# lizuoyue/torch-ngp

Measured on AMD Instinct MI355X. Metric: train-step rays/sec (fwd+bwd) on 800×800 Lego; 1/2/4/8 MI355X, higher is better.
Workload: dtype fp16

## Files before the change

torch-ngp_amd/csrc/ngp_head.h:

```cpp
#pragma once
#include "ngp_common.h"
#include "ngp_step.h"

#include <cfloat>


namespace ngp_head {

using ngp_step::StepState;

constexpr int kMaxBoxes = 8;
constexpr int kMaxTensors = 8;
constexpr uint32_t kMaxMapRes = 128;

NGP_DEV uint32_t mix32(uint32_t x) {
    x ^= x >> 16; x *= 0x7feb352du;
    x ^= x >> 15; x *= 0x846ca68bu;
    x ^= x >> 16;
    return x;
}
NGP_DEV uint32_t rng_u32(uint32_t seed, uint32_t a, uint32_t b, uint32_t c) {
    return mix32(seed ^ mix32(a + 0x9e3779b9u * mix32(b ^ mix32(c + 0x85ebca6bu))));
}
NGP_DEV float rng_unit(uint32_t seed, uint32_t a, uint32_t b, uint32_t c) {
// ... 311 lines not shown
#else
    const uint2 w = __builtin_bit_cast(uint2, g);
    return ((w.x | w.y) & 0x7fff7fffu) == 0u && m.x == 0.0f && m.y == 0.0f && m.z == 0.0f && m.w == 0.0f &&
           v.x == 0.0f && v.y == 0.0f && v.z == 0.0f && v.w == 0.0f;
#endif
}
constexpr uint32_t kAdamThreads = 256, kAdamChunk = kAdamThreads * 8;
template <int U = 2>
NGP_DEV void adam_sweep(const TensorList& tl, StepState* __restrict__ st, const AdamArgs& aa, uint32_t blk,
                        uint32_t nblk, uint32_t tid) {
    constexpr uint32_t kChunk = kAdamThreads * 4 * U;
    const ngp_step::AdamConsts ac = ngp_step::adam_consts(st, aa.base_lr, aa.beta1, aa.beta2, aa.iters,
                                                          aa.grad_mult);
    const bool skip = st->found_inf != 0 || ac.inv_bad;
    if (blk == 0 && tid == 0) {
        if (ac.inv_bad) st->found_inf = 1;
        if (aa.defer_end) st->end_pending = 1;
    }
    typedef _Float16 half4 __attribute__((ext_vector_type(4)));
    const bool shadow_all = (aa.zero_grads & 2) != 0;
    auto adam1 = [&](float& p, float& m, float& v, float gh) {
        ngp_step::adam_update(p, m, v, gh, ac, aa.beta1, aa.beta2, aa.eps);
    };
    const uint64_t total = tl.start[tl.n];
    const uint64_t nchunks = (total + kChunk - 1) / kChunk;
    for (uint64_t c = blk; c < nchunks; c += nblk) {
        const uint64_t c0 = c * kChunk, c1 = min(c0 + kChunk, total);
        const int k = find_tensor(tl, c0);
        if (find_tensor(tl, c1 - 1) == k && c1 - tl.start[k] <= tl.size[k]) {
            const uint64_t base = c0 - tl.start[k] + tid * 4;
            float4 pv[U], mv[U], vv[U];
            half4 gh[U];
            bool in[U];
#pragma unroll
            for (int u = 0; u < U; ++u) {
                const uint64_t off = base + u * (kChunk / U);
                in[u] = c0 + (off - (c0 - tl.start[k])) < c1;
                const uint64_t lo = in[u] ? off : c0 - tl.start[k];
                pv[u] = *reinterpret_cast<const float4*>(tl.p[k] + lo);
                mv[u] = *reinterpret_cast<const float4*>(tl.m[k] + lo);
                vv[u] = *reinterpret_cast<const float4*>(tl.v[k] + lo);
                gh[u] = *reinterpret_cast<const half4*>(tl.g[k] + lo);
            }
#pragma unroll
            for (int u = 0; u < U; ++u) {
                if (!in[u]) continue;
                const uint64_t off = base + u * (kChunk / U);
                const bool upd = !skip && !adam_idle(mv[u], vv[u], gh[u]);
                if (upd) {
                    adam1(pv[u].x, mv[u].x, vv[u].x, (float)gh[u][0]);
                    adam1(pv[u].y, mv[u].y, vv[u].y, (float)gh[u][1]);
                    adam1(pv[u].z, mv[u].z, vv[u].z, (float)gh[u][2]);
                    adam1(pv[u].w, mv[u].w, vv[u].w, (float)gh[u][3]);
                    *reinterpret_cast<float4*>(tl.p[k] + off) = pv[u];
                    *reinterpret_cast<float4*>(tl.m[k] + off) = mv[u];
                    *reinterpret_cast<float4*>(tl.v[k] + off) = vv[u];
                }
                if (tl.ph[k] && (upd || shadow_all))
                    *reinterpret_cast<half4*>(tl.ph[k] + off) =
                        half4{(ngp_half)pv[u].x, (ngp_half)pv[u].y, (ngp_half)pv[u].z, (ngp_half)pv[u].w};
                if (aa.zero_grads && grad_set(gh[u])) *reinterpret_cast<half4*>(tl.g[k] + off) = half4{0, 0, 0, 0};
            }
            continue;
        }
        for (uint64_t i = c0 + tid; i < c1; i += kAdamThreads) {
            const int kk = find_tensor(tl, i);
            const uint64_t off = i - tl.start[kk];
            if (off >= tl.size[kk]) continue;
            float p = tl.p[kk][off];
            if (!skip) {
                float m = tl.m[kk][off], v = tl.v[kk][off];
                adam1(p, m, v, (float)tl.g[kk][off]);
                tl.p[kk][off] = p;
                tl.m[kk][off] = m;
                tl.v[kk][off] = v;
            }
            if (tl.ph[kk] && (!skip || shadow_all)) tl.ph[kk][off] = (ngp_half)p;
            if (aa.zero_grads) tl.g[kk][off] = (ngp_half)0.0f;
        }
    }
}

template <int U>
NGP_DEV void adam_sweep_pipe(const TensorList& tl, StepState* __restrict__ st, const AdamArgs& aa, uint32_t blk,
                             uint32_t nblk, uint32_t tid) {
    constexpr uint32_t kChunk = kAdamThreads * 4 * U;
    typedef _Float16 half4 __attribute__((ext_vector_type(4)));
    const ngp_step::AdamConsts ac = ngp_step::adam_consts(st, aa.base_lr, aa.beta1, aa.beta2, aa.iters,
                                                          aa.grad_mult);
    const bool skip = st->found_inf != 0 || ac.inv_bad;
    if (blk == 0 && tid == 0) {
        if (ac.inv_bad) st->found_inf = 1;
        if (aa.defer_end) st->end_pending = 1;
    }
    const bool shadow_all = (aa.zero_grads & 2) != 0;
    const uint64_t total = tl.start[tl.n];
    const uint64_t nchunks = (total + kChunk - 1) / kChunk;
    struct Buf {
        float4 p[U], m[U], v[U];
        half4 g[U];
    };
    auto whole = [&](uint64_t c) {
        const uint64_t c0 = c * kChunk, c1 = min(c0 + kChunk, total);
        const int k = find_tensor(tl, c0);
        return find_tensor(tl, c1 - 1) == k && c1 - tl.start[k] <= tl.size[k] ? k : -1;
    };
    auto ld_f4 = [](const float* q) { return *reinterpret_cast<const float4*>(q); };
    auto st_f4 = [](float* q, float4 x) { *reinterpret_cast<float4*>(q) = x; };
    auto load = [&](uint64_t c, int k, Buf& b) {
        const uint64_t c0 = c * kChunk, c1 = min(c0 + kChunk, total), first = c0 - tl.start[k];
#pragma unroll
        for (int u = 0; u < U; ++u) {
            const uint64_t off = first + tid * 4 + u * (kChunk / U);
            const uint64_t lo = off + tl.start[k] < c1 ? off : first;
            b.p[u] = ld_f4(tl.p[k] + lo);
            b.m[u] = ld_f4(tl.m[k] + lo);
            b.v[u] = ld_f4(tl.v[k] + lo);
            b.g[u] = *reinterpret_cast<const half4*>(tl.g[k] + lo);
        }
    };
    auto apply = [&](uint64_t c, int k, Buf& b) {
        const uint64_t c0 = c * kChunk, c1 = min(c0 + kChunk, total), first = c0 - tl.start[k];
#pragma unroll
        for (int u = 0; u < U; ++u) {
            const uint64_t off = first + tid * 4 + u * (kChunk / U);
            if (off + tl.start[k] >= c1) continue;
            const bool upd = !skip && !adam_idle(b.m[u], b.v[u], b.g[u]);
            if (upd) {
                ngp_step::adam_update(b.p[u].x, b.m[u].x, b.v[u].x, (float)b.g[u][0], ac, aa.beta1, aa.beta2, aa.eps);
                ngp_step::adam_update(b.p[u].y, b.m[u].y, b.v[u].y, (float)b.g[u][1], ac, aa.beta1, aa.beta2, aa.eps);
                ngp_step::adam_update(b.p[u].z, b.m[u].z, b.v[u].z, (float)b.g[u][2], ac, aa.beta1, aa.beta2, aa.eps);
                ngp_step::adam_update(b.p[u].w, b.m[u].w, b.v[u].w, (float)b.g[u][3], ac, aa.beta1, aa.beta2, aa.eps);
                st_f4(tl.p[k] + off, b.p[u]);
                st_f4(tl.m[k] + off, b.m[u]);
                st_f4(tl.v[k] + off, b.v[u]);
            }
            if (tl.ph[k] && (upd || shadow_all))
                *reinterpret_cast<half4*>(tl.ph[k] + off) =
                    half4{(ngp_half)b.p[u].x, (ngp_half)b.p[u].y, (ngp_half)b.p[u].z, (ngp_half)b.p[u].w};
            if (aa.zero_grads && grad_set(b.g[u])) *reinterpret_cast<half4*>(tl.g[k] + off) = half4{0, 0, 0, 0};
        }
    };
    auto seam = [&](uint64_t c) {
        const uint64_t c0 = c * kChunk, c1 = min(c0 + kChunk, total);
        for (uint64_t i = c0 + tid; i < c1; i += kAdamThreads) {
            const int kk = find_tensor(tl, i);
            const uint64_t off = i - tl.start[kk];
            if (off >= tl.size[kk]) continue;
            float p = tl.p[kk][off];
            if (!skip) {
                float m = tl.m[kk][off], v = tl.v[kk][off];
                ngp_step::adam_update(p, m, v, (float)tl.g[kk][off], ac, aa.beta1, aa.beta2, aa.eps);
                tl.p[kk][off] = p;
                tl.m[kk][off] = m;
                tl.v[kk][off] = v;
            }
            if (tl.ph[kk] && (!skip || shadow_all)) tl.ph[kk][off] = (ngp_half)p;
            if (aa.zero_grads) tl.g[kk][off] = (ngp_half)0.0f;
        }
    };
    auto at = [](uint64_t i) { return i; };
    Buf a{}, b{};
    uint64_t c = blk;
    int ka = c < nchunks ? whole(at(c)) : -1;
    if (ka >= 0) load(at(c), ka, a);
    while (c < nchunks) {
        const uint64_t cn = c + nblk;
        const int kb = cn < nchunks ? whole(at(cn)) : -1;
        if (kb >= 0) load(at(cn), kb, b);
        if (ka >= 0) apply(at(c), ka, a);
        else seam(at(c));
        a = b;
        ka = kb;
        c = cn;
    }
}

}
```

torch-ngp_amd/csrc/raymarching.hip:

```cpp
#include "ffmlp_pack.h"
#include "ngp_common.h"
#include "ngp_dpp.h"
#include "ngp_head.h"
#include "ngp_render.h"
#include "ngp_step.h"

#include <algorithm>
#include <cfloat>

namespace {

constexpr float kSQRT3 = 1.7320508075688772f;
constexpr float kRPI = 0.3183098861837907f;

NGP_DEV float clampf(float x, float lo, float hi) { return fminf(hi, fmaxf(lo, x)); }
NGP_DEV float signf(float x) { return copysignf(1.0f, x); }

NGP_DEV int frexp_level(float mx, int max_level) {
    int e = 0;
    if (mx != 0.0f) e = (int)((__float_as_uint(mx) >> 23) & 0xffu) - 126;
    return min(max_level, max(0, e));
}

NGP_DEV uint32_t expand_bits(uint32_t v) {
// ... 504 lines not shown
    if (mine && off < k.max_steps) {
        float tj = ta;
        uint64_t m = mine;
        for (uint32_t j = 0; m && off < k.max_steps; ++j, tj = ch.step(tj)) {
            if ((m >> j) & 1ull) {
                ts[off++] = tj;
                m &= m - 1;
            }
        }
    }
    return total < k.max_steps ? total : k.max_steps;
}

template <bool ONE_LEVEL, typename OCC>
NGP_DEV uint32_t march_ray_wave(const Ray& r, const MarchConst& k, const OCC& occ, float t0, float far,
                                float* __restrict__ ts) {
    if (!(t0 < far)) return 0;
    if (k.dt_gamma == 0.0f) {
        const float delta = clampf(0.0f, k.dt_min, k.dt_max);
        const float ulp_far = __uint_as_float(((__float_as_uint(far) >> 23) & 0xffu) << 23) * 1.1920929e-7f;
        const double smin = (double)delta - (double)ulp_far;
        if (smin > 0.0) {
            const double kest = ceil(((double)far - (double)t0) / smin) + 2.0;
            const uint32_t L = (uint32_t)ceil(kest / 64.0);
            if (L <= 64) return march_ray_segmented<ONE_LEVEL>(r, k, occ, ChainConst{t0, delta}, far, L, ts);
        }
    } else if (k.dt_gamma > 0.0f) {
        ChainGamma ch;
        ch.k = k;
        const uint32_t K = chain_records(t0, far, k, ch.rec);
        if (K != kInf) {
            ch.nrec = ngp_div_up(K, kRecStride);
            const uint32_t L = kRecStride * ngp_div_up(ngp_div_up(K, 64u), kRecStride);
            return march_ray_segmented<ONE_LEVEL>(r, k, occ, ch, far, L > 0 ? L : kRecStride, ts);
        }
    }
    uint32_t n = 0;
    if ((threadIdx.x & 63) == 0) n = march_ray_train<ONE_LEVEL>(r, k, occ, t0, far, ts);
    return (uint32_t)__builtin_amdgcn_readlane((int)n, 0);
}

NGP_DEV void emit_sample(const float* __restrict__ rays_o, const float* __restrict__ rays_d, const MarchConst& k,
                         const float* __restrict__ nears, const float* __restrict__ noises,
                         const float* __restrict__ ts, uint32_t rn, uint32_t kk, size_t p, float* __restrict__ xyzs,
                         float* __restrict__ dirs, float* __restrict__ deltas) {
    const float* row = ts + (size_t)rn * k.max_steps;
    const float t = row[kk];
    const float tp = row[kk ? kk - 1 : 0u];
    const float nr = nears[rn], nz = noises[rn];
    const float prev = kk == 0 ? ray_t0(nr, nz, k) : tp + clampf(tp * k.dt_gamma, k.dt_min, k.dt_max);
    const float ox = rays_o[rn * 3], oy = rays_o[rn * 3 + 1], oz = rays_o[rn * 3 + 2];
    const float dx = rays_d[rn * 3], dy = rays_d[rn * 3 + 1], dz = rays_d[rn * 3 + 2];
    const float dt = clampf(t * k.dt_gamma, k.dt_min, k.dt_max);
    xyzs[p * 3 + 0] = clampf(fmaf(t, dx, ox), -k.bound, k.bound);
    xyzs[p * 3 + 1] = clampf(fmaf(t, dy, oy), -k.bound, k.bound);
    xyzs[p * 3 + 2] = clampf(fmaf(t, dz, oz), -k.bound, k.bound);
    dirs[p * 3 + 0] = dx;
    dirs[p * 3 + 1] = dy;
    dirs[p * 3 + 2] = dz;
    deltas[p * 2 + 0] = dt;
    deltas[p * 2 + 1] = (t + dt) - prev;
}

struct MarchAdam {
    ngp_head::TensorList tl;
    ngp_head::AdamArgs aa;
    ngp_step::StepState* st;
    uint4* clear;
    uint32_t clear16;
    bool emit_launch;
};
constexpr uint32_t kMarchAdamWaves = 4;

constexpr uint32_t kEmitMaxBlockRays = 64;
struct MarchEmit {
    uint32_t* ticket;
    uint32_t* error;
    unsigned long long* words;
    int32_t* counter;
    float *xyzs, *dirs, *deltas;
    uint32_t M, rb;
};

NGP_DEV unsigned long long agent_load_u64(const unsigned long long* p) {
    return __hip_atomic_load(p, __ATOMIC_RELAXED, __HIP_MEMORY_SCOPE_AGENT);
}

template <uint32_t MW>
__global__ void __launch_bounds__(kSegThreads)
k_march_train(const float* __restrict__ rays_o, const float* __restrict__ rays_d,
              const uint8_t* __restrict__ grid, const uint8_t* __restrict__ img, OccLayout L,
              MarchConst k, uint32_t N, const float* __restrict__ nears, const float* __restrict__ fars,
              const float* __restrict__ noises, int32_t* __restrict__ rays, float* __restrict__ ts,
              const int32_t* __restrict__ counter, uint32_t* __restrict__ scan, MarchAdam ma, MarchEmit me) {
    extern __shared__ uint4 dyn[];
    __shared__ uint32_t s_ticket, s_base0, s_arrive, s_ready, s_first;
    __shared__ uint32_t s_off[kEmitMaxBlockRays + 1];
    const bool emit = me.ticket != nullptr;
    if (blockIdx.x == 0 && threadIdx.x == 0) scan[0] = (uint32_t)counter[0];
    if (emit && threadIdx.x == 0) {
        s_ticket = atomicAdd(me.ticket, 1u);
        s_base0 = (uint32_t)counter[0];
        s_arrive = 0;
        s_ready = 0;
    }
    uint32_t* sum = reinterpret_cast<uint32_t*>(dyn);
    uint32_t* pre = sum + 4 * L.ngroups;
    const bool lds = L.ngroups > 0 && load_occ_index(img, L, dyn);
    if (emit) __syncthreads();
    const uint32_t wave = threadIdx.x >> 6;
    if (MW < kSegWaves && wave >= MW) {
        constexpr uint32_t kVirt = (kSegWaves - MW) / 4;
        if (blockIdx.x == 0 && wave == MW)
            for (uint32_t i = threadIdx.x & 63u; i < ma.clear16; i += 64) ma.clear[i] = uint4{0u, 0u, 0u, 0u};
        ngp_head::adam_sweep_pipe<2>(ma.tl, ma.st, ma.aa, blockIdx.x * kVirt + (wave - MW) / 4,
                                                    gridDim.x * kVirt, threadIdx.x & 255u);
        return;
    }
    const OccLds occ_lds{sum, pre, reinterpret_cast<const uint8_t*>(pre + L.ngroups)};
    const OccGlobal occ_glb{grid};
    const uint32_t G = gridDim.x;
    const uint32_t rank = emit ? s_ticket % G : blockIdx.x, epoch1 = emit ? s_ticket / G + 1u : 0u;
    const uint32_t n0 = emit ? rank * me.rb : 0u, n1 = emit ? min(N, n0 + me.rb) : N;
    const uint32_t lane = threadIdx.x & 63;
    for (uint32_t n = emit ? n0 + wave : blockIdx.x * MW + wave; n < n1; n += emit ? MW : G * MW) {
        const Ray r = load_ray(rays_o, rays_d, n);
        const float t0 = ray_t0(nears[n], noises[n], k);
        const float far = fars[n];
        float* row = ts + (size_t)n * k.max_steps;
        uint32_t cnt;
        if (lds) {
            cnt = k.C == 1 ? march_ray_wave<true>(r, k, occ_lds, t0, far, row)
                           : march_ray_wave<false>(r, k, occ_lds, t0, far, row);
        } else {
            cnt = k.C == 1 ? march_ray_wave<true>(r, k, occ_glb, t0, far, row)
                           : march_ray_wave<false>(r, k, occ_glb, t0, far, row);
        }
        if (lane == 0) {
            rays[n * 3 + 0] = (int32_t)n;
            rays[n * 3 + 2] = (int32_t)cnt;
            scan[4 + n] = cnt;
            if (emit) s_off[n - n0] = cnt;
        }
    }
    if (!emit) return;
    asm volatile("s_waitcnt vmcnt(0) lgkmcnt(0)" ::: "memory");
    __builtin_amdgcn_fence(__ATOMIC_RELEASE, "workgroup");
    uint32_t last = 0;
    if (lane == 0) last = atomicAdd(&s_arrive, 1u) == MW - 1 ? 1u : 0u;
    last = (uint32_t)__builtin_amdgcn_readfirstlane((int)last);
    const uint32_t nb = n1 > n0 ? n1 - n0 : 0u;
    if (last) {
        __builtin_amdgcn_fence(__ATOMIC_ACQUIRE, "workgroup");
        const uint32_t c = lane < nb ? s_off[lane] : 0u;
        uint32_t incl = c;
#pragma unroll
        for (uint32_t o = 1; o < 64; o <<= 1) {
            const uint32_t u = __shfl_up(incl, o, 64);
            if (lane >= o) incl += u;
        }
        const uint32_t total = (uint32_t)__builtin_amdgcn_readlane((int)incl, 63);
        if (lane == 0)
            __hip_atomic_store(me.words + rank, ((unsigned long long)epoch1 << 32) | total, __ATOMIC_RELAXED,
                               __HIP_MEMORY_SCOPE_AGENT);
        uint32_t part = 0;
        bool lost = false;
        for (uint32_t p = lane; p < rank; p += 64) {
            unsigned long long v = agent_load_u64(me.words + p);
            for (uint32_t spin = 0; (uint32_t)(v >> 32) != epoch1 && spin < (1u << 20); ++spin) {
                __builtin_amdgcn_s_sleep(2);
                v = agent_load_u64(me.words + p);
            }
            lost |= (uint32_t)(v >> 32) != epoch1;
            part += (uint32_t)v;
        }
        if (__ballot(lost) && lane == 0) atomicOr(me.error, 1u);
#pragma unroll
        for (uint32_t o = 32; o > 0; o >>= 1) part += __shfl_xor(part, o, 64);
        if (lane < nb) s_off[lane] = incl - c;
        if (lane == 0) {
            s_off[nb] = total;
            s_first = s_base0 + part;
            if (rank == G - 1) {
                me.counter[0] = (int32_t)(s_base0 + part + total);
                me.counter[1] += (int32_t)N;
            }
        }
        __builtin_amdgcn_fence(__ATOMIC_RELEASE, "workgroup");
        if (lane == 0) __hip_atomic_store(&s_ready, 1u, __ATOMIC_RELAXED, __HIP_MEMORY_SCOPE_WORKGROUP);
    } else {
        for (uint32_t spin = 0; __hip_atomic_load(&s_ready, __ATOMIC_RELAXED, __HIP_MEMORY_SCOPE_WORKGROUP) == 0u &&
                                spin < (1u << 22); ++spin)
            __builtin_amdgcn_s_sleep(1);
        if (__hip_atomic_load(&s_ready, __ATOMIC_RELAXED, __HIP_MEMORY_SCOPE_WORKGROUP) == 0u && lane == 0)
            atomicOr(me.error, 2u);
        __builtin_amdgcn_fence(__ATOMIC_ACQUIRE, "workgroup");
    }
    const uint32_t base = s_first, btotal = s_off[nb];
    const uint32_t t = threadIdx.x;
    for (uint32_t i = t; i < nb; i += 64 * MW) rays[(size_t)(n0 + i) * 3 + 1] = (int32_t)(base + s_off[i]);
    for (uint32_t j = t; j < btotal; j += 64 * MW) {
        uint32_t lo = 0, hi = nb;
        while (hi - lo > 1) {
            const uint32_t mid = (lo + hi) >> 1;
            if (s_off[mid] <= j) lo = mid; else hi = mid;
        }
        if (base + s_off[lo + 1] > me.M) continue;
        emit_sample(rays_o, rays_d, k, nears, noises, ts, n0 + lo, j - s_off[lo], (size_t)base + j, me.xyzs,
                    me.dirs, me.deltas);
    }
}
static_assert((kSegWaves - kMarchAdamWaves) % 4 == 0, "Adam waves form 256-thread virtual blocks");

struct EmitTail {
    ngp_step::StepState* st;
    bool end;
    ngp_step::ScalerArgs sa;
    const float* loss_ray;
    uint32_t n_rays, groups;
    ngp_pack::PackJobs jobs;
};

__global__ void __launch_bounds__(kMarchThreads)
k_march_emit(const float* __restrict__ rays_o, const float* __restrict__ rays_d, MarchConst k,
             uint32_t N, uint32_t M, const float* __restrict__ nears, const float* __restrict__ noises,
             const float* __restrict__ ts, float* __restrict__ xyzs, float* __restrict__ dirs,
             float* __restrict__ deltas, int32_t* __restrict__ rays, const uint32_t* __restrict__ scan,
             int32_t* __restrict__ counter, EmitTail tail) {
    const bool has_tail = tail.st != nullptr;
    if (has_tail && blockIdx.y == 0) {
        if (blockIdx.x == 0) {
            if (tail.end && tail.st->end_pending)
                ngp_step::step_end_block(tail.st, tail.sa, nullptr, nullptr, tail.loss_ray, tail.n_rays);
        } else if (blockIdx.x - 1 < (uint32_t)tail.jobs.n) {
            const ngp_pack::PackJob& j = tail.jobs.job[blockIdx.x - 1];
            ngp_pack::build_frags(j.image, j.w, j.m, j.transposed != 0);
        }
        return;
    }
    if (blockIdx.x >= tail.groups) return;
    __shared__ uint32_t off[kMarchThreads + 1];
    __shared__ uint32_t lds_waves[kMarchThreads / 64];
    const uint32_t* __restrict__ counts = scan + 4;
    const uint32_t n0 = blockIdx.x * kMarchThreads;
    uint32_t part = 0;
    for (uint32_t i0 = threadIdx.x; i0 < n0; i0 += 8 * kMarchThreads) {
        uint32_t v[8];
#pragma unroll
        for (int u = 0; u < 8; ++u) {
            const uint32_t i = i0 + u * kMarchThreads;
            v[u] = counts[i < n0 ? i : 0u];
        }
#pragma unroll
        for (int u = 0; u < 8; ++u) part += i0 + u * kMarchThreads < n0 ? v[u] : 0u;
    }
    uint32_t before;
    block_exclusive_scan<kMarchThreads>(part, lds_waves, before);
    const uint32_t base = scan[0] + before;
    const uint32_t n = n0 + threadIdx.x;
    const uint32_t c = n < N ? counts[n] : 0u;
    uint32_t total;
    const uint32_t excl = block_exclusive_scan<kMarchThreads>(c, lds_waves, total);
    off[threadIdx.x] = excl;
    if (threadIdx.x == 0) off[kMarchThreads] = total;
    const uint32_t ey = blockIdx.y - (has_tail ? 1u : 0u);
    if (ey == 0) {
        if (n < N) rays[(size_t)n * 3 + 1] = (int32_t)(base + excl);
        if (blockIdx.x == tail.groups - 1 && threadIdx.x == 0) {
            counter[0] = (int32_t)(base + total);
            counter[1] += (int32_t)N;
        }
    }
    __syncthreads();

    const uint32_t chunk = ngp_div_up(total, kEmitSplit);
    const uint32_t j0 = ey * chunk, j1 = min(total, j0 + chunk);
    for (uint32_t j = j0 + threadIdx.x; j < j1; j += kMarchThreads) {
        uint32_t lo = 0, hi = kMarchThreads;
        while (hi - lo > 1) {
            const uint32_t mid = (lo + hi) >> 1;
            if (off[mid] <= j) lo = mid; else hi = mid;
        }
        const uint32_t rn = n0 + lo, kk = j - off[lo];
        if (base + off[lo + 1] > M) continue;
        emit_sample(rays_o, rays_d, k, nears, noises, ts, rn, kk, (size_t)base + j, xyzs, dirs, deltas);
    }
}

OccLayout occ_layout(const uint8_t* grid, uint32_t C, uint32_t H) {
    OccLayout L{};
    const size_t nbytes = (size_t)C * H * H * H / 8;
    L.nbytes = (uint32_t)nbytes;
// ... 384 lines not shown
    if (N == 0) return NGP_OK;
    NGP_REQUIRE((reinterpret_cast<uintptr_t>(grid) & 15) == 0, NGP_ERR_ARG, "packbits: grid must be 16-byte aligned");
    k_packbits<<<ngp_div_up(N, 256), 256, 0, ngp_stream(stream)>>>(grid, N, density_thresh, bitfield);
    return ngp_check_launch("packbits");
}

static size_t march_ts_bytes(uint32_t N, uint32_t max_steps) {
    return ((size_t)N * max_steps * sizeof(float) + 255) / 256 * 256;
}
static size_t march_scan_bytes(uint32_t N) { return ((size_t)(N + 4) * sizeof(uint32_t) + 255) / 256 * 256; }

static size_t march_sync_bytes() { return 256 + 8 * (size_t)kMaxMarchBlocks; }

extern "C" size_t ngp_march_rays_train_workspace_bytes(uint32_t N, uint32_t max_steps, uint32_t C,
                                                        uint32_t H) {
    OccLayout L = occ_layout(nullptr, C, H);
    return march_ts_bytes(N, max_steps) + march_scan_bytes(N) + (occ_image_bytes(L) + occ_scratch_bytes(L) + 255) /
           256 * 256 + march_sync_bytes();
}

extern "C" size_t ngp_march_rays_train_error_offset(uint32_t N, uint32_t max_steps, uint32_t C, uint32_t H) {
    const OccLayout L = occ_layout(nullptr, C, H);
    return march_ts_bytes(N, max_steps) + march_scan_bytes(N) +
           (occ_image_bytes(L) + occ_scratch_bytes(L) + 255) / 256 * 256 + 4;
}


static int march_train_impl(const float* rays_o, const float* rays_d, const uint8_t* grid,
                             float bound, float dt_gamma, uint32_t max_steps, uint32_t N, uint32_t C,
                             uint32_t H, uint32_t M, const float* nears, const float* fars,
                             float* xyzs, float* dirs, float* deltas, int32_t* rays, int32_t* counter,
                             const float* noises, void* workspace, size_t workspace_bytes,
                             bool build_image, void* stream, const EmitTail* tail = nullptr,
                             const MarchAdam* ma = nullptr) {
    if (int e = check_cascade(C, H, max_steps)) return e;
    NGP_REQUIRE(rays && counter, NGP_ERR_ARG, "march_rays_train: null rays/counter");
    if (N == 0) return NGP_OK;
    const size_t need = ngp_march_rays_train_workspace_bytes(N, max_steps, C, H);
    NGP_REQUIRE(workspace && workspace_bytes >= need, NGP_ERR_ARG,
                "march_rays_train: workspace of %zu bytes required, got %zu", need, workspace_bytes);
    NGP_REQUIRE((reinterpret_cast<uintptr_t>(workspace) & 15) == 0, NGP_ERR_ARG,
                "march_rays_train: workspace must be 16-byte aligned");
    const MarchConst k = make_march_const(bound, dt_gamma, max_steps, C, H);
    const OccLayout L = occ_layout(grid, C, H);
    hipStream_t st = ngp_stream(stream);
    const uint32_t groups = ngp_div_up(N, kMarchThreads);
    const uint32_t wgs = ngp_div_up(N, kSegWaves);
    const uint32_t blocks = wgs < kMaxMarchBlocks ? wgs : kMaxMarchBlocks;
    float* ts = static_cast<float*>(workspace);
    uint32_t* scan = reinterpret_cast<uint32_t*>(static_cast<uint8_t*>(workspace) + march_ts_bytes(N, max_steps));
    uint8_t* img = reinterpret_cast<uint8_t*>(scan) + march_scan_bytes(N);
    if (L.ngroups && build_image) {
        uint32_t* cnt = reinterpret_cast<uint32_t*>(img + occ_image_bytes(L));
        const uint32_t wg = ngp_div_up(L.ngroups, kBuildThreads);
        k_occ_count<<<wg, kBuildThreads, 0, st>>>(grid, L, img, cnt);
        k_occ_compact<<<ngp_div_up(L.ngroups, kCompactGroups), kBuildThreads, 0, st>>>(grid, L, img, cnt);
    }
    MarchEmit me{};
    if (ma && ma->st) {
        const uint32_t rb = ngp_div_up(N, kMaxMarchBlocks);
        if (rb <= kEmitMaxBlockRays && !ma->emit_launch) {
            uint8_t* sync = img + (occ_image_bytes(L) + occ_scratch_bytes(L) + 255) / 256 * 256;
            me = MarchEmit{reinterpret_cast<uint32_t*>(sync), reinterpret_cast<uint32_t*>(sync) + 1,
                           reinterpret_cast<unsigned long long*>(sync + 256), counter, xyzs, dirs, deltas, M, rb};
        }
        k_march_train<kMarchAdamWaves><<<kMaxMarchBlocks, kSegThreads, L.ngroups ? kMarchLdsBytes : 0, st>>>(
            rays_o, rays_d, grid, img, L, k, N, nears, fars, noises, rays, ts, counter, scan, *ma, me);
    } else {
        k_march_train<kSegWaves><<<blocks, kSegThreads, L.ngroups ? kMarchLdsBytes : 0, st>>>(
            rays_o, rays_d, grid, img, L, k, N, nears, fars, noises, rays, ts, counter, scan, MarchAdam{},
            MarchEmit{});
    }
    if (me.ticket && !tail) return ngp_check_launch("march_rays_train");
    EmitTail et{};
    if (tail) et = *tail;
    et.groups = me.ticket ? 0u : groups;
    const uint32_t gx = tail ? std::max<uint32_t>(et.groups, 1u + (uint32_t)tail->jobs.n) : groups;
    const uint32_t gy = me.ticket ? 1u : kEmitSplit + (tail ? 1u : 0u);
    k_march_emit<<<dim3(gx, gy), kMarchThreads, 0, st>>>(rays_o, rays_d, k, N, M, nears, noises, ts, xyzs, dirs,
                                                         deltas, rays, scan, counter, et);
    return ngp_check_launch("march_rays_train");
}

extern "C" int ngp_march_rays_train(const float* rays_o, const float* rays_d, const uint8_t* grid,
                                    float bound, float dt_gamma, uint32_t max_steps, uint32_t N,
                                    uint32_t C, uint32_t H, uint32_t M, const float* nears,
                                    const float* fars, float* xyzs, float* dirs, float* deltas,
                                    int32_t* rays, int32_t* counter, const float* noises,
                                    void* workspace, size_t workspace_bytes, void* stream) {
    return march_train_impl(rays_o, rays_d, grid, bound, dt_gamma, max_steps, N, C, H, M, nears, fars,
                            xyzs, dirs, deltas, rays, counter, noises, workspace, workspace_bytes, true,
                            stream);
}

extern "C" int ngp_march_occupancy_build(const uint8_t* grid, uint32_t C, uint32_t H, uint32_t N,
                                         uint32_t max_steps, void* workspace, size_t workspace_bytes,
                                         void* stream) {
    if (int e = check_cascade(C, H, max_steps)) return e;
    const size_t need = ngp_march_rays_train_workspace_bytes(N, max_steps, C, H);
    NGP_REQUIRE(workspace && workspace_bytes >= need, NGP_ERR_ARG,
                "march_occupancy_build: workspace of %zu bytes required, got %zu", need, workspace_bytes);
    const OccLayout L = occ_layout(grid, C, H);
    if (!L.ngroups) return NGP_OK;
    hipStream_t st = ngp_stream(stream);
    uint8_t* img = static_cast<uint8_t*>(workspace) + march_ts_bytes(N, max_steps) + march_scan_bytes(N);
    uint32_t* cnt = reinterpret_cast<uint32_t*>(img + occ_image_bytes(L));
    const uint32_t wg = ngp_div_up(L.ngroups, kBuildThreads);
    k_occ_count<<<wg, kBuildThreads, 0, st>>>(grid, L, img, cnt);
    k_occ_compact<<<ngp_div_up(L.ngroups, kCompactGroups), kBuildThreads, 0, st>>>(grid, L, img, cnt);
    return ngp_check_launch("march_occupancy_build");
}

extern "C" int ngp_march_rays_train_prebuilt(const float* rays_o, const float* rays_d,
                                             const uint8_t* grid, float bound, float dt_gamma,
                                             uint32_t max_steps, uint32_t N, uint32_t C, uint32_t H,
                                             uint32_t M, const float* nears, const float* fars,
                                             float* xyzs, float* dirs, float* deltas, int32_t* rays,
                                             int32_t* counter, const float* noises, void* workspace,
                                             size_t workspace_bytes, void* stream) {
    return march_train_impl(rays_o, rays_d, grid, bound, dt_gamma, max_steps, N, C, H, M, nears, fars,
                            xyzs, dirs, deltas, rays, counter, noises, workspace, workspace_bytes, false,
                            stream);
}

extern "C" int ngp_march_rays_train_prebuilt_tail(const float* rays_o, const float* rays_d,
                                                  const uint8_t* grid, float bound, float dt_gamma,
                                                  uint32_t max_steps, uint32_t N, uint32_t C, uint32_t H,
                                                  uint32_t M, const float* nears, const float* fars,
                                                  float* xyzs, float* dirs, float* deltas, int32_t* rays,
                                                  int32_t* counter, const float* noises, void* workspace,
                                                  size_t workspace_bytes, void* state, float growth_factor,
                                                  float backoff_factor, int32_t growth_interval,
                                                  int32_t scaler_enabled, const float* loss_ray, int32_t n_nets,
                                                  const void* const* mlp_weights, const uint32_t* in_dims,
                                                  const uint32_t* hidden_dims, const uint32_t* num_layers,
                                                  void* const* images, void* stream) {
    NGP_REQUIRE(state && loss_ray, NGP_ERR_ARG, "march_rays_train_prebuilt_tail: null state or loss_ray");
    EmitTail tail{};
    tail.st = static_cast<ngp_step::StepState*>(state);
    tail.end = true;
    tail.sa = ngp_step::ScalerArgs{growth_factor, backoff_factor, growth_interval, scaler_enabled,
                                   N ? 1.0f / (float)N : 0.0f};
    tail.loss_ray = loss_ray;
    tail.n_rays = N;
    if (n_nets > 0)
        if (int e = ngp_pack::build_jobs(n_nets, mlp_weights, in_dims, hidden_dims, num_layers, images, tail.jobs))
            return e;
    return march_train_impl(rays_o, rays_d, grid, bound, dt_gamma, max_steps, N, C, H, M, nears, fars,
                            xyzs, dirs, deltas, rays, counter, noises, workspace, workspace_bytes, false,
                            stream, &tail);
}

extern "C" int ngp_march_rays_train_prebuilt_adam(const float* rays_o, const float* rays_d,
                                                  const uint8_t* grid, float bound, float dt_gamma,
                                                  uint32_t max_steps, uint32_t N, uint32_t C, uint32_t H,
                                                  uint32_t M, const float* nears, const float* fars,
                                                  float* xyzs, float* dirs, float* deltas, int32_t* rays,
                                                  int32_t* counter, const float* noises, void* workspace,
                                                  size_t workspace_bytes, void* state, float growth_factor,
                                                  float backoff_factor, int32_t growth_interval,
                                                  int32_t scaler_enabled, const float* loss_ray, int32_t n_nets,
                                                  const void* const* mlp_weights, const uint32_t* in_dims,
                                                  const uint32_t* hidden_dims, const uint32_t* num_layers,
                                                  void* const* images, const ngp_adam_job* job, void* stream) {
    NGP_REQUIRE(state && loss_ray && job, NGP_ERR_ARG, "march_rays_train_prebuilt_adam: null state, loss_ray or job");
    NGP_REQUIRE(job->n_tensors >= 1 && job->n_tensors <= ngp_head::kMaxTensors, NGP_ERR_ARG,
// ... 130 lines not shown
```

Measured before the change: 29.59 million.

## Let march waves join fused Adam sweep via per-block dynamic slice stealing

```diff
diff --git a/torch-ngp_amd/csrc/ngp_head.h b/torch-ngp_amd/csrc/ngp_head.h
--- a/torch-ngp_amd/csrc/ngp_head.h
+++ b/torch-ngp_amd/csrc/ngp_head.h
@@ -417,24 +417,23 @@
 }
 
 template <int U>
-NGP_DEV void adam_sweep_pipe(const TensorList& tl, StepState* __restrict__ st, const AdamArgs& aa, uint32_t blk,
-                             uint32_t nblk, uint32_t tid) {
+NGP_DEV uint32_t adam_sweep_pipe(const TensorList& tl, StepState* __restrict__ st, const AdamArgs& aa, uint32_t wg,
+                                 uint32_t nwg, uint32_t virt, int32_t first, uint32_t* next, bool head) {
     constexpr uint32_t kChunk = kAdamThreads * 4 * U;
     typedef _Float16 half4 __attribute__((ext_vector_type(4)));
-    const ngp_step::AdamConsts ac = ngp_step::adam_consts(st, aa.base_lr, aa.beta1, aa.beta2, aa.iters,
-                                                          aa.grad_mult);
-    const bool skip = st->found_inf != 0 || ac.inv_bad;
-    if (blk == 0 && tid == 0) {
-        if (ac.inv_bad) st->found_inf = 1;
-        if (aa.defer_end) st->end_pending = 1;
-    }
-    const bool shadow_all = (aa.zero_grads & 2) != 0;
+    const uint32_t lane = threadIdx.x & 63u;
     const uint64_t total = tl.start[tl.n];
     const uint64_t nchunks = (total + kChunk - 1) / kChunk;
     struct Buf {
         float4 p[U], m[U], v[U];
         half4 g[U];
     };
+    struct Slot {
+        uint64_t c;
+        uint32_t tid;
+        int k;
+        bool ok;
+    };
     auto whole = [&](uint64_t c) {
         const uint64_t c0 = c * kChunk, c1 = min(c0 + kChunk, total);
         const int k = find_tensor(tl, c0);
@@ -442,23 +441,54 @@
     };
     auto ld_f4 = [](const float* q) { return *reinterpret_cast<const float4*>(q); };
     auto st_f4 = [](float* q, float4 x) { *reinterpret_cast<float4*>(q) = x; };
-    auto load = [&](uint64_t c, int k, Buf& b) {
-        const uint64_t c0 = c * kChunk, c1 = min(c0 + kChunk, total), first = c0 - tl.start[k];
+    auto load = [&](const Slot& s, Buf& b) {
+        const uint64_t c0 = s.c * kChunk, c1 = min(c0 + kChunk, total), first_el = c0 - tl.start[s.k];
 #pragma unroll
         for (int u = 0; u < U; ++u) {
-            const uint64_t off = first + tid * 4 + u * (kChunk / U);
-            const uint64_t lo = off + tl.start[k] < c1 ? off : first;
-            b.p[u] = ld_f4(tl.p[k] + lo);
-            b.m[u] = ld_f4(tl.m[k] + lo);
-            b.v[u] = ld_f4(tl.v[k] + lo);
-            b.g[u] = *reinterpret_cast<const half4*>(tl.g[k] + lo);
-        }
-    };
-    auto apply = [&](uint64_t c, int k, Buf& b) {
-        const uint64_t c0 = c * kChunk, c1 = min(c0 + kChunk, total), first = c0 - tl.start[k];
+            const uint64_t off = first_el + s.tid * 4 + u * (kChunk / U);
+            const uint64_t lo = off + tl.start[s.k] < c1 ? off : first_el;
+            b.p[u] = ld_f4(tl.p[s.k] + lo);
+            b.m[u] = ld_f4(tl.m[s.k] + lo);
+            b.v[u] = ld_f4(tl.v[s.k] + lo);
+            b.g[u] = *reinterpret_cast<const half4*>(tl.g[s.k] + lo);
+        }
+    };
+    const uint64_t per_round = (uint64_t)nwg * virt;
+    const uint32_t rounds = (uint32_t)((nchunks + per_round - 1) / per_round);
+    auto fetch = [&](uint32_t s, Slot& x, Buf& b) {
+        const uint32_t w = s % (4 * virt), rr = s / (4 * virt);
+        x.ok = rr < rounds;
+        const uint32_t round = !x.ok ? 0u : rr < 2 ? rounds - 1 - rr : rr - 2;
+        x.c = (uint64_t)round * per_round + (uint64_t)wg * virt + w / 4;
+        x.tid = (w % 4) * 64 + lane;
+        x.k = x.ok && x.c < nchunks ? whole(x.c) : -2;
+        if (x.k >= 0) load(x, b);
+    };
+    auto take = [&]() {
+        uint32_t v = 0;
+        if (lane == 0) v = atomicAdd(next, 1u);
+        return v;
+    };
+    auto taken = [](uint32_t v) { return (uint32_t)__builtin_amdgcn_readfirstlane((int)v); };
+    Slot s0{0, 0, -2, false}, s1{0, 0, -2, false};
+    Buf b0{}, b1{};
+    fetch(first >= 0 ? (uint32_t)first : taken(take()), s0, b0);
+    uint32_t ahead = s0.ok ? take() : 0u;
+
+    const ngp_step::AdamConsts ac = ngp_step::adam_consts(st, aa.base_lr, aa.beta1, aa.beta2, aa.iters,
+                                                          aa.grad_mult);
+    const bool skip = st->found_inf != 0 || ac.inv_bad;
+    if (head && lane == 0) {
+        if (ac.inv_bad) st->found_inf = 1;
+        if (aa.defer_end) st->end_pending = 1;
+    }
+    const bool shadow_all = (aa.zero_grads & 2) != 0;
+    auto apply = [&](const Slot& s, Buf& b) {
+        const int k = s.k;
+        const uint64_t c0 = s.c * kChunk, c1 = min(c0 + kChunk, total), first_el = c0 - tl.start[k];
 #pragma unroll
         for (int u = 0; u < U; ++u) {
-            const uint64_t off = first + tid * 4 + u * (kChunk / U);
+            const uint64_t off = first_el + s.tid * 4 + u * (kChunk / U);
             if (off + tl.start[k] >= c1) continue;
             const bool upd = !skip && !adam_idle(b.m[u], b.v[u], b.g[u]);
             if (upd) {
@@ -476,39 +506,56 @@
             if (aa.zero_grads && grad_set(b.g[u])) *reinterpret_cast<half4*>(tl.g[k] + off) = half4{0, 0, 0, 0};
         }
     };
-    auto seam = [&](uint64_t c) {
-        const uint64_t c0 = c * kChunk, c1 = min(c0 + kChunk, total);
-        for (uint64_t i = c0 + tid; i < c1; i += kAdamThreads) {
-            const int kk = find_tensor(tl, i);
-            const uint64_t off = i - tl.start[kk];
-            if (off >= tl.size[kk]) continue;
-            float p = tl.p[kk][off];
-            if (!skip) {
-                float m = tl.m[kk][off], v = tl.v[kk][off];
-                ngp_step::adam_update(p, m, v, (float)tl.g[kk][off], ac, aa.beta1, aa.beta2, aa.eps);
-                tl.p[kk][off] = p;
-                tl.m[kk][off] = m;
-                tl.v[kk][off] = v;
+    auto seam = [&](const Slot& s) {
+        constexpr int E = 2;
+        const uint64_t c0 = s.c * kChunk, c1 = min(c0 + kChunk, total);
+        const int ka = find_tensor(tl, c0), kb = find_tensor(tl, c1 - 1);
+        for (int t = ka; t <= kb; ++t) {
+            const uint64_t t0 = tl.start[t], t1 = t0 + tl.size[t];
+            if (t1 == t0) continue;
+            float *const tp = tl.p[t], *const tm = tl.m[t], *const tv = tl.v[t];
+            ngp_half *const tg = tl.g[t], *const th = tl.ph[t];
+            for (uint64_t i0 = c0 + s.tid; i0 < c1; i0 += (uint64_t)E * kAdamThreads) {
+                uint64_t off[E];
+                bool in[E];
+                float p[E], m[E], v[E];
+                ngp_half g[E];
+#pragma unroll
+                for (int e = 0; e < E; ++e) {
+                    const uint64_t i = i0 + (uint64_t)e * kAdamThreads;
+                    in[e] = i < c1 && i >= t0 && i < t1;
+                    off[e] = in[e] ? i - t0 : 0;
+                    p[e] = tp[off[e]];
+                    m[e] = tm[off[e]];
+                    v[e] = tv[off[e]];
+                    g[e] = tg[off[e]];
+                }
+#pragma unroll
+                for (int e = 0; e < E; ++e) {
+                    if (!in[e]) continue;
+                    if (!skip) {
+                        ngp_step::adam_update(p[e], m[e], v[e], (float)g[e], ac, aa.beta1, aa.beta2, aa.eps);
+                        tp[off[e]] = p[e];
+                        tm[off[e]] = m[e];
+                        tv[off[e]] = v[e];
+                    }
+                    if (th && (!skip || shadow_all)) th[off[e]] = (ngp_half)p[e];
+                    if (aa.zero_grads) tg[off[e]] = (ngp_half)0.0f;
+                }
             }
-            if (tl.ph[kk] && (!skip || shadow_all)) tl.ph[kk][off] = (ngp_half)p;
-            if (aa.zero_grads) tl.g[kk][off] = (ngp_half)0.0f;
-        }
-    };
-    auto at = [](uint64_t i) { return i; };
-    Buf a{}, b{};
-    uint64_t c = blk;
-    int ka = c < nchunks ? whole(at(c)) : -1;
-    if (ka >= 0) load(at(c), ka, a);
-    while (c < nchunks) {
-        const uint64_t cn = c + nblk;
-        const int kb = cn < nchunks ? whole(at(cn)) : -1;
-        if (kb >= 0) load(at(cn), kb, b);
-        if (ka >= 0) apply(at(c), ka, a);
-        else seam(at(c));
-        a = b;
-        ka = kb;
-        c = cn;
-    }
-}
-
-}
+        }
+    };
+    uint32_t swept = 0;
+    while (s0.ok) {
+        fetch(taken(ahead), s1, b1);
+        if (s1.ok) ahead = take();
+        if (s0.k >= 0) apply(s0, b0);
+        else if (s0.k == -1) seam(s0);
+        swept += s0.k != -2;
+        s0 = s1;
+        b0 = b1;
+    }
+    return swept;
+}
+
+}
diff --git a/torch-ngp_amd/csrc/raymarching.hip b/torch-ngp_amd/csrc/raymarching.hip
--- a/torch-ngp_amd/csrc/raymarching.hip
+++ b/torch-ngp_amd/csrc/raymarching.hip
@@ -610,6 +610,15 @@
     uint32_t M, rb;
 };
 
+#ifdef NGP_STAMPS
+__device__ unsigned long long* g_march_stamps;
+#define ASTAMPV(slot, v) do { if (g_march_stamps && (threadIdx.x & 63) == 0) g_march_stamps[((size_t)blockIdx.x * kSegWaves + (threadIdx.x >> 6)) * 8 + (slot)] = (v); } while (0)
+#define ASTAMP(slot) ASTAMPV(slot, __builtin_amdgcn_s_memrealtime())
+#else
+#define ASTAMPV(slot, v) do { } while (0)
+#define ASTAMP(slot) do { } while (0)
+#endif
+
 NGP_DEV unsigned long long agent_load_u64(const unsigned long long* p) {
     return __hip_atomic_load(p, __ATOMIC_RELAXED, __HIP_MEMORY_SCOPE_AGENT);
 }
@@ -622,28 +631,59 @@
               const float* __restrict__ noises, int32_t* __restrict__ rays, float* __restrict__ ts,
               const int32_t* __restrict__ counter, uint32_t* __restrict__ scan, MarchAdam ma, MarchEmit me) {
     extern __shared__ uint4 dyn[];
-    __shared__ uint32_t s_ticket, s_base0, s_arrive, s_ready, s_first;
+    __shared__ uint32_t s_ticket, s_base0, s_arrive, s_ready, s_first, s_slice;
     __shared__ uint32_t s_off[kEmitMaxBlockRays + 1];
     const bool emit = me.ticket != nullptr;
+    const uint32_t wave = threadIdx.x >> 6;
+    constexpr uint32_t kVirt = MW < kSegWaves ? (kSegWaves - MW) / 4 : 1;
     if (blockIdx.x == 0 && threadIdx.x == 0) scan[0] = (uint32_t)counter[0];
-    if (emit && threadIdx.x == 0) {
-        s_ticket = atomicAdd(me.ticket, 1u);
-        s_base0 = (uint32_t)counter[0];
-        s_arrive = 0;
-        s_ready = 0;
-    }
     uint32_t* sum = reinterpret_cast<uint32_t*>(dyn);
     uint32_t* pre = sum + 4 * L.ngroups;
-    const bool lds = L.ngroups > 0 && load_occ_index(img, L, dyn);
-    if (emit) __syncthreads();
-    const uint32_t wave = threadIdx.x >> 6;
-    if (MW < kSegWaves && wave >= MW) {
-        constexpr uint32_t kVirt = (kSegWaves - MW) / 4;
-        if (blockIdx.x == 0 && wave == MW)
-            for (uint32_t i = threadIdx.x & 63u; i < ma.clear16; i += 64) ma.clear[i] = uint4{0u, 0u, 0u, 0u};
-        ngp_head::adam_sweep_pipe<2>(ma.tl, ma.st, ma.aa, blockIdx.x * kVirt + (wave - MW) / 4,
-                                                    gridDim.x * kVirt, threadIdx.x & 255u);
-        return;
+    bool lds;
+    if constexpr (MW < kSegWaves) {
+        ASTAMP(0);
+        if (threadIdx.x == 0) {
+            s_arrive = 0;
+            s_ready = 0;
+            s_slice = kSegWaves - MW;
+            if (emit) {
+                s_ticket = atomicAdd(me.ticket, 1u);
+                s_base0 = (uint32_t)counter[0];
+            }
+        }
+        uint64_t warm = ma.tl.start[1] ^ ma.tl.start[2] ^ ma.tl.size[0] ^ ma.tl.size[1];
+#pragma unroll
+        for (int q = 0; q < 2; ++q)
+            warm ^= reinterpret_cast<uintptr_t>(ma.tl.p[q]) ^ reinterpret_cast<uintptr_t>(ma.tl.m[q]) ^
+                    reinterpret_cast<uintptr_t>(ma.tl.v[q]) ^ reinterpret_cast<uintptr_t>(ma.tl.g[q]) ^
+                    reinterpret_cast<uintptr_t>(ma.tl.ph[q]);
+        lds = false;
+        if (L.ngroups > 0) {
+            const uint32_t total = reinterpret_cast<const uint32_t*>(img)[0];
+            lds = total <= L.cap;
+            if (lds) {
+                const uint32_t n16 = (20 * L.ngroups + total + 15) / 16;
+                const uint4* src = reinterpret_cast<const uint4*>(img + 16);
+#pragma unroll 8
+                for (uint32_t i = threadIdx.x; i < n16; i += kSegThreads) dyn[i] = src[i];
+            }
+        }
+        asm volatile("" ::"s"(warm));
+        asm volatile("s_waitcnt lgkmcnt(0)\n\ts_barrier" ::: "memory");
+        ASTAMP(1);
+        if (wave >= MW) {
+            if (blockIdx.x == 0 && wave == MW)
+                for (uint32_t i = threadIdx.x & 63u; i < ma.clear16; i += 64) ma.clear[i] = uint4{0u, 0u, 0u, 0u};
+            const uint32_t swept = ngp_head::adam_sweep_pipe<2>(ma.tl, ma.st, ma.aa, blockIdx.x, gridDim.x, kVirt,
+                                                                (int32_t)(wave - MW), &s_slice,
+                                                                blockIdx.x == 0 && wave == MW);
+            ASTAMP(4);
+            ASTAMPV(5, swept);
+            (void)swept;
+            return;
+        }
+    } else {
+        lds = L.ngroups > 0 && load_occ_index(img, L, dyn);
     }
     const OccLds occ_lds{sum, pre, reinterpret_cast<const uint8_t*>(pre + L.ngroups)};
     const OccGlobal occ_glb{grid};
@@ -671,71 +711,81 @@
             if (emit) s_off[n - n0] = cnt;
         }
     }
-    if (!emit) return;
-    asm volatile("s_waitcnt vmcnt(0) lgkmcnt(0)" ::: "memory");
-    __builtin_amdgcn_fence(__ATOMIC_RELEASE, "workgroup");
-    uint32_t last = 0;
-    if (lane == 0) last = atomicAdd(&s_arrive, 1u) == MW - 1 ? 1u : 0u;
-    last = (uint32_t)__builtin_amdgcn_readfirstlane((int)last);
-    const uint32_t nb = n1 > n0 ? n1 - n0 : 0u;
-    if (last) {
-        __builtin_amdgcn_fence(__ATOMIC_ACQUIRE, "workgroup");
-        const uint32_t c = lane < nb ? s_off[lane] : 0u;
-        uint32_t incl = c;
-#pragma unroll
-        for (uint32_t o = 1; o < 64; o <<= 1) {
-            const uint32_t u = __shfl_up(incl, o, 64);
-            if (lane >= o) incl += u;
-        }
-        const uint32_t total = (uint32_t)__builtin_amdgcn_readlane((int)incl, 63);
-        if (lane == 0)
-            __hip_atomic_store(me.words + rank, ((unsigned long long)epoch1 << 32) | total, __ATOMIC_RELAXED,
-                               __HIP_MEMORY_SCOPE_AGENT);
-        uint32_t part = 0;
-        bool lost = false;
-        for (uint32_t p = lane; p < rank; p += 64) {
-            unsigned long long v = agent_load_u64(me.words + p);
-            for (uint32_t spin = 0; (uint32_t)(v >> 32) != epoch1 && spin < (1u << 20); ++spin) {
-                __builtin_amdgcn_s_sleep(2);
-                v = agent_load_u64(me.words + p);
+    if (MW < kSegWaves) ASTAMP(2);
+    if (emit) {
+        asm volatile("s_waitcnt vmcnt(0) lgkmcnt(0)" ::: "memory");
+        __builtin_amdgcn_fence(__ATOMIC_RELEASE, "workgroup");
+        uint32_t last = 0;
+        if (lane == 0) last = atomicAdd(&s_arrive, 1u) == MW - 1 ? 1u : 0u;
+        last = (uint32_t)__builtin_amdgcn_readfirstlane((int)last);
+        const uint32_t nb = n1 > n0 ? n1 - n0 : 0u;
+        if (last) {
+            __builtin_amdgcn_fence(__ATOMIC_ACQUIRE, "workgroup");
+            const uint32_t c = lane < nb ? s_off[lane] : 0u;
+            uint32_t incl = c;
+    #pragma unroll
+            for (uint32_t o = 1; o < 64; o <<= 1) {
+                const uint32_t u = __shfl_up(incl, o, 64);
+                if (lane >= o) incl += u;
             }
-            lost |= (uint32_t)(v >> 32) != epoch1;
-            part += (uint32_t)v;
-        }
-        if (__ballot(lost) && lane == 0) atomicOr(me.error, 1u);
-#pragma unroll
-        for (uint32_t o = 32; o > 0; o >>= 1) part += __shfl_xor(part, o, 64);
-        if (lane < nb) s_off[lane] = incl - c;
-        if (lane == 0) {
-            s_off[nb] = total;
-            s_first = s_base0 + part;
-            if (rank == G - 1) {
-                me.counter[0] = (int32_t)(s_base0 + part + total);
-                me.counter[1] += (int32_t)N;
+            const uint32_t total = (uint32_t)__builtin_amdgcn_readlane((int)incl, 63);
+            if (lane == 0)
+                __hip_atomic_store(me.words + rank, ((unsigned long long)epoch1 << 32) | total, __ATOMIC_RELAXED,
+                                   __HIP_MEMORY_SCOPE_AGENT);
+            uint32_t part = 0;
+            bool lost = false;
+            for (uint32_t p = lane; p < rank; p += 64) {
+                unsigned long long v = agent_load_u64(me.words + p);
+                for (uint32_t spin = 0; (uint32_t)(v >> 32) != epoch1 && spin < (1u << 20); ++spin) {
+                    __builtin_amdgcn_s_sleep(2);
+                    v = agent_load_u64(me.words + p);
+                }
+                lost |= (uint32_t)(v >> 32) != epoch1;
+                part += (uint32_t)v;
             }
-        }
-        __builtin_amdgcn_fence(__ATOMIC_RELEASE, "workgroup");
-        if (lane == 0) __hip_atomic_store(&s_ready, 1u, __ATOMIC_RELAXED, __HIP_MEMORY_SCOPE_WORKGROUP);
-    } else {
-        for (uint32_t spin = 0; __hip_atomic_load(&s_ready, __ATOMIC_RELAXED, __HIP_MEMORY_SCOPE_WORKGROUP) == 0u &&
-                                spin < (1u << 22); ++spin)
-            __builtin_amdgcn_s_sleep(1);
-        if (__hip_atomic_load(&s_ready, __ATOMIC_RELAXED, __HIP_MEMORY_SCOPE_WORKGROUP) == 0u && lane == 0)
-            atomicOr(me.error, 2u);
-        __builtin_amdgcn_fence(__ATOMIC_ACQUIRE, "workgroup");
-    }
-    const uint32_t base = s_first, btotal = s_off[nb];
-    const uint32_t t = threadIdx.x;
-    for (uint32_t i = t; i < nb; i += 64 * MW) rays[(size_t)(n0 + i) * 3 + 1] = (int32_t)(base + s_off[i]);
-    for (uint32_t j = t; j < btotal; j += 64 * MW) {
-        uint32_t lo = 0, hi = nb;
-        while (hi - lo > 1) {
-            const uint32_t mid = (lo + hi) >> 1;
-            if (s_off[mid] <= j) lo = mid; else hi = mid;
-        }
-        if (base + s_off[lo + 1] > me.M) continue;
-        emit_sample(rays_o, rays_d, k, nears, noises, ts, n0 + lo, j - s_off[lo], (size_t)base + j, me.xyzs,
-                    me.dirs, me.deltas);
+            if (__ballot(lost) && lane == 0) atomicOr(me.error, 1u);
+    #pragma unroll
+            for (uint32_t o = 32; o > 0; o >>= 1) part += __shfl_xor(part, o, 64);
+            if (lane < nb) s_off[lane] = incl - c;
+            if (lane == 0) {
+                s_off[nb] = total;
+                s_first = s_base0 + part;
+                if (rank == G - 1) {
+                    me.counter[0] = (int32_t)(s_base0 + part + total);
+                    me.counter[1] += (int32_t)N;
+                }
+            }
+            __builtin_amdgcn_fence(__ATOMIC_RELEASE, "workgroup");
+            if (lane == 0) __hip_atomic_store(&s_ready, 1u, __ATOMIC_RELAXED, __HIP_MEMORY_SCOPE_WORKGROUP);
+        } else {
+            for (uint32_t spin = 0; __hip_atomic_load(&s_ready, __ATOMIC_RELAXED, __HIP_MEMORY_SCOPE_WORKGROUP) == 0u &&
+                                    spin < (1u << 22); ++spin)
+                __builtin_amdgcn_s_sleep(1);
+            if (__hip_atomic_load(&s_ready, __ATOMIC_RELAXED, __HIP_MEMORY_SCOPE_WORKGROUP) == 0u && lane == 0)
+                atomicOr(me.error, 2u);
+            __builtin_amdgcn_fence(__ATOMIC_ACQUIRE, "workgroup");
+        }
+        const uint32_t base = s_first, btotal = s_off[nb];
+        const uint32_t t = threadIdx.x;
+        for (uint32_t i = t; i < nb; i += 64 * MW) rays[(size_t)(n0 + i) * 3 + 1] = (int32_t)(base + s_off[i]);
+        for (uint32_t j = t; j < btotal; j += 64 * MW) {
+            uint32_t lo = 0, hi = nb;
+            while (hi - lo > 1) {
+                const uint32_t mid = (lo + hi) >> 1;
+                if (s_off[mid] <= j) lo = mid; else hi = mid;
+            }
+            if (base + s_off[lo + 1] > me.M) continue;
+            emit_sample(rays_o, rays_d, k, nears, noises, ts, n0 + lo, j - s_off[lo], (size_t)base + j, me.xyzs,
+                        me.dirs, me.deltas);
+        }
+    if (MW < kSegWaves) ASTAMP(3);
+    }
+    if constexpr (MW < kSegWaves) {
+        const uint32_t swept = ngp_head::adam_sweep_pipe<2>(
+            ma.tl, ma.st, ma.aa, blockIdx.x, gridDim.x, kVirt, -1, &s_slice, false);
+        ASTAMP(4);
+        ASTAMPV(5, swept);
+        (void)swept;
     }
 }
 static_assert((kSegWaves - kMarchAdamWaves) % 4 == 0, "Adam waves form 256-thread virtual blocks");
@@ -1286,6 +1336,12 @@
     return ngp_check_launch("march_rays_train");
 }
 
+#ifdef NGP_STAMPS
+extern "C" int ngp_debug_march_stamps(void* buf) {
+    return hipMemcpyToSymbol(HIP_SYMBOL(g_march_stamps), &buf, sizeof(buf)) == hipSuccess ? NGP_OK : NGP_ERR_HIP;
+}
+#endif
+
 extern "C" int ngp_march_rays_train(const float* rays_o, const float* rays_d, const uint8_t* grid,
                                     float bound, float dt_gamma, uint32_t max_steps, uint32_t N,
                                     uint32_t C, uint32_t H, uint32_t M, const float* nears,
```

Result: no change. 29.43 million (-0.5%).
